# jiaozihao18/LC-Rec

Hardware: NVIDIA B200
Metric: items indexed/sec (4-level RQ + Sinkhorn collision resolution) (higher is better)
Workload: dtype f32

## Files before the change

include/lcrec_b200.h:

```cpp
#ifndef LCREC_B200_H
#define LCREC_B200_H

#include <stddef.h>
#include <stdint.h>

#ifdef __cplusplus
extern "C" {
#endif

#define LCREC_OK 0
#define LCREC_ERR_ARG 1
#define LCREC_ERR_CUDA 2
#define LCREC_ERR_UNSUPPORTED 3
#define LCREC_ERR_NOMEM 4
#define LCREC_ERR_NUMERIC 5

#define LCREC_MAX_LEVELS 8

int lcrec_version(void);
const char* lcrec_strerror(int code);
const char* lcrec_last_error(void);
int lcrec_device_check(void);

typedef struct lcrec_mlp lcrec_mlp_t;
// ... 135 lines not shown
                                        void* stream);
int lcrec_sort_codes(const int64_t* codes, int64_t n, int n_levels, const int32_t* n_codes,
                     uint64_t* keys_out, uint32_t* items_out, void* ws, int64_t ws_bytes, void* stream);

typedef struct lcrec_indexer lcrec_indexer_t;
int lcrec_indexer_create(lcrec_mlp_t* encoder, int e_dim, int n_levels, const float* const* codebooks,
                         const int32_t* n_codes, double last_epsilon, int sk_iters,
                         int64_t max_items, int64_t chunk_rows, lcrec_indexer_t** out);
int lcrec_indexer_destroy(lcrec_indexer_t* ix);
int lcrec_indexer_run_device(lcrec_indexer_t* ix, const float* x, int64_t n, int max_rounds,
                             int64_t* codes, int64_t* stats_host, void* stream);
int lcrec_indexer_run_host(lcrec_indexer_t* ix, const float* x_host, int64_t n, int max_rounds,
                           int64_t* codes_host, int64_t* stats_host, void* stream);
int lcrec_indexer_run_device_ex(lcrec_indexer_t* ix, const void* x, int dtype, int64_t n, int max_rounds,
                                int64_t* codes, int64_t* stats_host, void* stream);
int lcrec_indexer_run_host_ex(lcrec_indexer_t* ix, const void* x_host, int dtype, int64_t n, int max_rounds,
                              int64_t* codes_host, int64_t* stats_host, void* stream);
int lcrec_indexer_pass0(lcrec_indexer_t* ix, const float* x, int64_t n, int64_t row_offset, void* stream);
int lcrec_indexer_pass0_ex(lcrec_indexer_t* ix, const void* x, int dtype, int64_t n, int64_t row_offset, void* stream);
int lcrec_indexer_round(lcrec_indexer_t* ix, int64_t n, int64_t* counts_host, void* stream);
int lcrec_indexer_resolve(lcrec_indexer_t* ix, int64_t* codes, const float* resid, int64_t n, int max_rounds,
                          int64_t* stats_host, void* stream);
int lcrec_indexer_set_segments(int on);
int lcrec_indexer_set_speculative(int on);
int64_t* lcrec_indexer_codes(lcrec_indexer_t* ix);
float* lcrec_indexer_resid(lcrec_indexer_t* ix);
int64_t lcrec_kmeans_workspace_bytes(int64_t n, int e_dim, int n_codes);
int lcrec_kmeans_center(const float* x, int64_t n, int e_dim, float* xc, float* mean, double* mean_variance_host,
                        void* workspace, int64_t workspace_bytes, void* stream);
int lcrec_kmeans_lloyd(const float* xc, int64_t n, int e_dim, float* centers, int n_codes, int max_iter, double tol,
                       const float* add_mean, int64_t* labels_out, double* inertia_host, int* n_iter_host,
                       void* workspace, int64_t workspace_bytes, void* stream);
int64_t lcrec_kmeanspp_workspace_bytes(int64_t n, int n_trials);
int lcrec_kmeanspp_seed(const float* xc, int64_t n, int e_dim, int n_clusters, int64_t first_index, const double* draws,
                        int n_trials, int64_t* indices, float* centers, void* workspace, int64_t workspace_bytes,
                        void* stream);
int lcrec_ema_update(const float* latent, const int64_t* indices, int64_t n, int n_codes, int e_dim,
                     double ema_decay, double epsilon, float* cluster_size, float* ema_w, float* codebook,
                     void* stream);
int lcrec_codebook_usage(const float* cluster_size, int n_codes, double epsilon, double reset_threshold,
                         int64_t* used_codes, uint8_t* unused_mask, void* stream);
int64_t lcrec_masked_mean_pool_workspace_bytes(int64_t n_seq, int64_t seq_len, int hidden_dim);
int lcrec_masked_mean_pool(const void* hidden, int dtype, const int64_t* mask, int64_t n_seq, int64_t seq_len,
                           int hidden_dim, float* out, int64_t out_stride, int accumulate, double divide_by,
                           void* workspace, int64_t workspace_bytes, void* stream);
int64_t lcrec_index_json_workspace_bytes(int64_t n);
// ... 25 lines not shown
```

lcrec_b200/_lib.py:

```python
from __future__ import annotations

import ctypes as C
import os

_HERE = os.path.dirname(os.path.abspath(__file__))
LIB_PATH = os.path.join(_HERE, "liblcrec_b200.so")

i32, i64, f64 = C.c_int32, C.c_int64, C.c_double
vp = C.c_void_p
pp = C.POINTER(C.c_void_p)

SIGNATURES = {
    "lcrec_version": (C.c_int, []),
    "lcrec_strerror": (C.c_char_p, [C.c_int]),
    "lcrec_last_error": (C.c_char_p, []),
    "lcrec_device_check": (C.c_int, []),
    "lcrec_launch_count": (i64, []),
    "lcrec_mlp_create": (C.c_int, [C.c_int, C.POINTER(i32), pp, pp, C.c_int, vp, pp]),
    "lcrec_mlp_update": (C.c_int, [vp, pp, pp, vp]),
    "lcrec_mlp_destroy": (C.c_int, [vp]),
    "lcrec_mlp_workspace_bytes": (i64, [vp, i64]),
    "lcrec_mlp_forward": (C.c_int, [vp, vp, i64, vp, pp, vp, i64, vp]),
    "lcrec_mlp_forward_ex": (C.c_int, [vp, vp, C.c_int, i64, vp, pp, vp, i64, vp]),
    "lcrec_mlp_set_acc_chunk": (C.c_int, [vp, C.c_int]),
# ... 31 lines not shown
                                           C.c_int, C.c_int, C.c_int, vp, vp, i64, vp]),
    "lcrec_sinkhorn_set_mode": (C.c_int, [C.c_int]),
    "lcrec_collisions_workspace_bytes": (i64, [i64]),
    "lcrec_collisions": (C.c_int, [vp, i64, C.c_int, C.POINTER(i32), vp, vp, vp, vp, i64, vp]),
    "lcrec_sort_codes": (C.c_int, [vp, i64, C.c_int, C.POINTER(i32), vp, vp, vp, i64, vp]),
    "lcrec_prefix_segments": (C.c_int, [vp, i64, C.c_int, C.POINTER(i32), vp, vp, vp, vp, i64, vp]),
    "lcrec_segment_collisions_workspace_bytes": (i64, [i64]),
    "lcrec_collisions_in_segments": (C.c_int, [vp, i64, C.c_int, C.c_int, vp, vp, vp, i64, vp, vp, vp, vp, i64, vp]),
    "lcrec_collisions_in_segments_active": (C.c_int, [vp, i64, C.c_int, C.c_int, vp, vp, vp, i64, vp, vp, vp, vp, vp, vp, vp, vp,
                                                      i64, vp]),
    "lcrec_profile_enable": (C.c_int, [C.c_int]),
    "lcrec_profile_collect": (C.c_int, [C.POINTER(C.c_double), C.POINTER(i64)]),
    "lcrec_indexer_create": (C.c_int, [vp, C.c_int, C.c_int, pp, C.POINTER(i32), f64, C.c_int, i64, i64, pp]),
    "lcrec_indexer_destroy": (C.c_int, [vp]),
    "lcrec_indexer_run_device": (C.c_int, [vp, vp, i64, C.c_int, vp, C.POINTER(i64), vp]),
    "lcrec_indexer_run_host": (C.c_int, [vp, vp, i64, C.c_int, vp, C.POINTER(i64), vp]),
    "lcrec_indexer_pass0": (C.c_int, [vp, vp, i64, i64, vp]),
    "lcrec_indexer_run_device_ex": (C.c_int, [vp, vp, C.c_int, i64, C.c_int, vp, C.POINTER(i64), vp]),
    "lcrec_indexer_run_host_ex": (C.c_int, [vp, vp, C.c_int, i64, C.c_int, vp, C.POINTER(i64), vp]),
    "lcrec_indexer_pass0_ex": (C.c_int, [vp, vp, C.c_int, i64, i64, vp]),
    "lcrec_indexer_round": (C.c_int, [vp, i64, C.POINTER(i64), vp]),
    "lcrec_indexer_resolve": (C.c_int, [vp, vp, vp, i64, C.c_int, C.POINTER(i64), vp]),
    "lcrec_indexer_set_segments": (C.c_int, [C.c_int]),
    "lcrec_indexer_set_speculative": (C.c_int, [C.c_int]),
    "lcrec_ema_update": (C.c_int, [vp, vp, i64, C.c_int, C.c_int, f64, f64, vp, vp, vp, vp]),
    "lcrec_codebook_usage": (C.c_int, [vp, C.c_int, f64, f64, vp, vp, vp]),
    "lcrec_masked_mean_pool_workspace_bytes": (i64, [i64, i64, C.c_int]),
    "lcrec_masked_mean_pool": (C.c_int, [vp, C.c_int, vp, i64, i64, C.c_int, vp, i64, C.c_int, f64, vp, i64, vp]),
    "lcrec_kmeans_workspace_bytes": (i64, [i64, C.c_int, C.c_int]),
    "lcrec_kmeans_center": (C.c_int, [vp, i64, C.c_int, vp, vp, C.POINTER(f64), vp, i64, vp]),
    "lcrec_kmeans_lloyd": (C.c_int, [vp, i64, C.c_int, vp, C.c_int, C.c_int, f64, vp, vp, C.POINTER(f64), C.POINTER(C.c_int),
                                     vp, i64, vp]),
    "lcrec_rq_train_forward": (C.c_int, [vp, vp, i64, C.c_int, C.c_int, pp, vp, vp, vp, vp, vp]),
    "lcrec_rq_train_backward": (C.c_int, [vp, vp, i64, C.c_int, C.c_int, C.POINTER(i32), vp, vp, f64, vp, pp, vp]),
    "lcrec_adam_workspace_bytes": (i64, [C.c_int, C.POINTER(i64)]),
    "lcrec_adam_clip_step": (C.c_int, [C.c_int, pp, pp, pp, pp, C.POINTER(i64), f64, f64, f64, f64, f64, C.c_int, i64, f64,
                                       C.c_int, vp, vp, i64, vp]),
    "lcrec_adam_hyper": (C.c_int, [f64, f64, f64, f64, i64, C.POINTER(C.c_float)]),
    "lcrec_adam_clip_step_dev": (C.c_int, [C.c_int, pp, pp, pp, pp, C.POINTER(i64), vp, f64, f64, f64, f64, C.c_int, f64,
                                           C.c_int, vp, vp, i64, vp]),
    "lcrec_simple_opt_clip_step": (C.c_int, [C.c_int, C.c_int, pp, pp, pp, C.POINTER(i64), f64, f64, f64, f64, f64, C.c_int, vp, vp, i64, vp]),
    "lcrec_bn_sums_elems": (i64, [C.c_int]),
    "lcrec_bn_splits": (C.c_int, [i64, C.c_int]),
    "lcrec_bn_forward_reduce": (C.c_int, [vp, i64, C.c_int, vp, vp]),
    "lcrec_bn_forward_apply": (C.c_int, [vp, vp, C.c_int, i64, i64, C.c_int, vp, vp, f64, f64, C.c_int, vp, vp, vp, vp, vp, vp]),
    "lcrec_bn_backward_reduce": (C.c_int, [vp, vp, vp, C.c_int, vp, vp, i64, C.c_int, vp, vp]),
# ... 64 lines not shown
```

lcrec_b200/build.py:

```python
from __future__ import annotations

import os
import subprocess
import sys

HERE = os.path.dirname(os.path.abspath(__file__))
CSRC = os.path.join(HERE, "csrc")
LIB = os.path.join(HERE, "liblcrec_b200.so")
SOURCES = ["abi.cu", "linear_tf32x3.cu", "linear_pair.cu", "rq_fused.cu", "sinkhorn.cu", "collide.cu", "ema.cu", "pool.cu", "kmeans.cu", "rq_train.cu", "optim.cu", "kmeanspp.cu", "train_extra.cu", "json_emit.cu", "sinkhorn_cluster.cu", "exchange.cu"]
NVCC_FLAGS = ["-O3", "-std=c++17", "-gencode", "arch=compute_100a,code=sm_100a", "-lineinfo",
              "-Xcompiler", "-fPIC", "--expt-relaxed-constexpr"]


def _stale() -> bool:
    if not os.path.exists(LIB):
        return True
    t = os.path.getmtime(LIB)
    deps = [os.path.join(CSRC, f) for f in os.listdir(CSRC)] + [os.path.join(HERE, "..", "include", "lcrec_b200.h")]
    return any(os.path.getmtime(d) > t for d in deps)


def build(force: bool = False, verbose: bool = False) -> str:
    if not force and not _stale():
        return LIB
    nvcc = os.environ.get("NVCC", "/usr/local/cuda/bin/nvcc")
    objs = []
    procs = []
    for src in SOURCES:
        obj = os.path.join(CSRC, src.replace(".cu", ".o"))
        objs.append(obj)
        cmd = [nvcc, *NVCC_FLAGS, "-c", os.path.join(CSRC, src), "-o", obj]
        if verbose:
# ... 19 lines not shown
```

lcrec_b200/csrc/abi.cu:

```cuda
#include <stdarg.h>
#include <string.h>

#include <utility>
#include <vector>

#include <nvtx3/nvToolsExt.h>

#include "common.cuh"

namespace lcrec {

static const char* stage_name(int tag) {
  static const char* mlp[] = {"lcrec/mlp_layer1", "lcrec/mlp_layer2", "lcrec/mlp_layer3", "lcrec/mlp_layer4", "lcrec/mlp_layer5",
                              "lcrec/mlp_layer6", "lcrec/mlp_layer7", "lcrec/mlp_layer8+"};
  if (tag == 0) return "lcrec/input_operand_split";
  if (tag >= 1 && tag <= 16) return mlp[tag - 1 < 7 ? tag - 1 : 7];
  switch (tag) {
    case 17: return "lcrec/tail_operand_splits";
    case 20: return "lcrec/rq_quantize";
    case 21: return "lcrec/collision_check";
    case 22: return "lcrec/sinkhorn_groups_round1";
    case 23: return "lcrec/sinkhorn_groups_later_rounds";
    case 24: return "lcrec/sinkhorn_warp_classes";
    case 26: return "lcrec/sinkhorn_literal_rerun";
    default: return "lcrec/stage";
  }
}

static thread_local char g_err[512] = "";
std::atomic<int64_t> g_launches{0};

void set_error(const char* fmt, ...) {
  va_list ap;
  va_start(ap, fmt);
  vsnprintf(g_err, sizeof(g_err), fmt, ap);
  va_end(ap);
}

int num_sms() {
  static int sms = -1;
  if (sms < 0) {
// ... 91 lines not shown
  lcrec_mlp_t* enc = nullptr;
  int in_dim = 0, D = 0, L = 0;
  std::vector<const float*> cb;
  std::vector<int32_t> K;
  double eps = 0.003; int iters = 50;
  int64_t max_items = 0, chunk_rows = 0;
  int64_t* codes = nullptr; float* resid = nullptr; float* z = nullptr;
  void* mlp_ws = nullptr; int64_t mlp_ws_bytes = 0;
  int64_t* offsets = nullptr; int64_t* members = nullptr; int64_t* counts = nullptr; int32_t* flags = nullptr;
  void* col_ws = nullptr; int64_t col_ws_bytes = 0;
  void* sk_ws = nullptr; int64_t sk_ws_bytes = 0;
  int64_t* seg_offsets = nullptr; int64_t* seg_members = nullptr; int64_t* seg_counts = nullptr;
  void* seg_ws = nullptr; int64_t seg_ws_bytes = 0;
  int32_t* seg_active[2] = {nullptr, nullptr}; int32_t* seg_active_count = nullptr;
  float* stage[2] = {nullptr, nullptr};
  int64_t* counts_host = nullptr;
  cudaStream_t copy_stream = nullptr;
  cudaEvent_t ev_copied[2] = {nullptr, nullptr}, ev_consumed[2] = {nullptr, nullptr};
  cudaStream_t round_stream = nullptr; cudaEvent_t round_ev = nullptr;
  cudaGraphExec_t round_exec[2] = {nullptr, nullptr};
  int64_t round_launches[2] = {0, 0};
  const int64_t* rg_codes = nullptr; const float* rg_resid = nullptr; int64_t rg_n = -1; int rg_key = -1;
  bool rg_failed = false;
};

extern "C" int lcrec_mlp_in_dim(const lcrec_mlp_t* m);
extern "C" int lcrec_mlp_out_dim(const lcrec_mlp_t* m);

#define IX_ALLOC(ptr, bytes)                                                                     \
  do {                                                                                           \
    if (cudaMalloc((void**)&(ptr), (size_t)(bytes)) != cudaSuccess) {                            \
      set_error("indexer: cudaMalloc(%lld) failed: %s", (long long)(bytes), cudaGetErrorString(cudaGetLastError())); \
      lcrec_indexer_destroy(ix);                                                                 \
      return LCREC_ERR_NOMEM;                                                                    \
    }                                                                                            \
  } while (0)

extern "C" int lcrec_indexer_create(lcrec_mlp_t* encoder, int e_dim, int n_levels, const float* const* codebooks,
                                    const int32_t* n_codes, double last_epsilon, int sk_iters, int64_t max_items,
                                    int64_t chunk_rows, lcrec_indexer_t** out) {
  LC_ARG(encoder && e_dim > 0 && n_levels >= 1 && n_levels <= LCREC_MAX_LEVELS && codebooks && n_codes && out);
  LC_ARG(max_items > 0 && chunk_rows > 0 && last_epsilon > 0.0 && sk_iters >= 0);
  LC_ARG(lcrec_mlp_out_dim(encoder) == e_dim);
  LC_TRY(lcrec_device_check());
  lcrec_indexer* ix = new lcrec_indexer();
  ix->enc = encoder; ix->in_dim = lcrec_mlp_in_dim(encoder); ix->D = e_dim; ix->L = n_levels;
// ... 4 lines not shown
  IX_ALLOC(ix->resid, sizeof(float) * max_items * e_dim);
  IX_ALLOC(ix->z, sizeof(float) * max_items * e_dim);
  ix->mlp_ws_bytes = lcrec_mlp_workspace_bytes(encoder, ix->chunk_rows);
  IX_ALLOC(ix->mlp_ws, ix->mlp_ws_bytes);
  IX_ALLOC(ix->offsets, sizeof(int64_t) * (max_items + 1));
  IX_ALLOC(ix->members, sizeof(int64_t) * max_items);
  IX_ALLOC(ix->counts, sizeof(int64_t) * 8);
  ix->flags = reinterpret_cast<int32_t*>(ix->counts + 4);
  ix->col_ws_bytes = lcrec_collisions_workspace_bytes(max_items);
  IX_ALLOC(ix->col_ws, ix->col_ws_bytes);
  ix->sk_ws_bytes = lcrec_sinkhorn_groups_workspace_bytes(max_items, n_codes[n_levels - 1]);
  IX_ALLOC(ix->sk_ws, ix->sk_ws_bytes);
  IX_ALLOC(ix->seg_offsets, sizeof(int64_t) * (max_items + 1));
  IX_ALLOC(ix->seg_members, sizeof(int64_t) * max_items);
  IX_ALLOC(ix->seg_counts, sizeof(int64_t) * 8);
  ix->seg_ws_bytes = lcrec_segment_collisions_workspace_bytes(max_items / 2 + 1);
  IX_ALLOC(ix->seg_ws, ix->seg_ws_bytes);
  IX_ALLOC(ix->seg_active[0], sizeof(int32_t) * (max_items / 2 + 2));
  IX_ALLOC(ix->seg_active[1], sizeof(int32_t) * (max_items / 2 + 2));
  IX_ALLOC(ix->seg_active_count, sizeof(int32_t) * 2);
  if (cudaMallocHost((void**)&ix->counts_host, sizeof(int64_t) * 8) != cudaSuccess) {
    set_error("indexer: cudaMallocHost failed"); lcrec_indexer_destroy(ix); return LCREC_ERR_NOMEM;
  }
  *out = ix;
  return LCREC_OK;
}

extern "C" int lcrec_indexer_destroy(lcrec_indexer_t* ix) {
  if (!ix) return LCREC_OK;
  cudaFree(ix->codes); cudaFree(ix->resid); cudaFree(ix->z); cudaFree(ix->mlp_ws); cudaFree(ix->offsets);
  cudaFree(ix->members); cudaFree(ix->counts); cudaFree(ix->col_ws); cudaFree(ix->sk_ws);
  cudaFree(ix->seg_offsets); cudaFree(ix->seg_members); cudaFree(ix->seg_counts); cudaFree(ix->seg_ws);
  cudaFree(ix->seg_active[0]); cudaFree(ix->seg_active[1]); cudaFree(ix->seg_active_count);
  cudaFree(ix->stage[0]); cudaFree(ix->stage[1]);
  if (ix->counts_host) cudaFreeHost(ix->counts_host);
  for (int i = 0; i < 2; ++i) { if (ix->ev_copied[i]) cudaEventDestroy(ix->ev_copied[i]); if (ix->ev_consumed[i]) cudaEventDestroy(ix->ev_consumed[i]); }
  if (ix->copy_stream) cudaStreamDestroy(ix->copy_stream);
  for (int i = 0; i < 2; ++i) if (ix->round_exec[i]) cudaGraphExecDestroy(ix->round_exec[i]);
  if (ix->round_ev) cudaEventDestroy(ix->round_ev);
  if (ix->round_stream) cudaStreamDestroy(ix->round_stream);
  delete ix;
  return LCREC_OK;
}

extern "C" int64_t* lcrec_indexer_codes(lcrec_indexer_t* ix) { return ix ? ix->codes : nullptr; }
extern "C" float* lcrec_indexer_resid(lcrec_indexer_t* ix) { return ix ? ix->resid : nullptr; }

extern "C" int lcrec_indexer_pass0_ex(lcrec_indexer_t* ix, const void* x, int dtype, int64_t n, int64_t row_offset, void* stream) {
  LC_ARG(dtype_ok(dtype));
  LC_ARG(ix && n >= 0 && row_offset >= 0 && row_offset + n <= ix->max_items);
  if (n == 0) return LCREC_OK;
  LC_ARG(x != nullptr);
  const int64_t row_bytes = dtype_bytes(dtype) * ix->in_dim;
  for (int64_t s = 0; s < n; s += ix->chunk_rows) {
    const int64_t m = std::min(ix->chunk_rows, n - s);
    LC_TRY(lcrec_mlp_forward_ex(ix->enc, static_cast<const char*>(x) + s * row_bytes, dtype, m, ix->z + s * ix->D, nullptr,
                                ix->mlp_ws, ix->mlp_ws_bytes, stream));
  }
  {
    ProfScope prof(20, (cudaStream_t)stream);
    LC_TRY(lcrec_rq_quantize(ix->z, n, ix->D, ix->L, ix->cb.data(), ix->K.data(), ix->L, ix->L - 1,
                             ix->codes + row_offset * ix->L, nullptr, ix->resid + row_offset * ix->D,
                             nullptr, stream));
  }
  return LCREC_OK;
}

extern "C" int lcrec_indexer_pass0(lcrec_indexer_t* ix, const float* x, int64_t n, int64_t row_offset, void* stream) {
  return lcrec_indexer_pass0_ex(ix, x, kDtypeF32, n, row_offset, stream);
}

static int g_use_segments = 1;
extern "C" int lcrec_indexer_set_segments(int on) { g_use_segments = on ? 1 : 0; return LCREC_OK; }

static int collide_and_fetch(lcrec_indexer_t* ix, const int64_t* codes, int64_t n, int seg_round, cudaStream_t st) {
  {
    ProfScope prof(21, st);
    if (seg_round >= 0) {
      const int in = (seg_round + 1) & 1, out = seg_round & 1;
      LC_CUDA(cudaMemsetAsync(ix->seg_active_count + out, 0, sizeof(int32_t), st));
      LC_TRY(lcrec_collisions_in_segments_active(codes, n, ix->L, ix->L - 1, ix->seg_offsets, ix->seg_members, ix->seg_counts + 1,
                                                 n / 2 + 1, seg_round > 0 ? ix->seg_active[in] : nullptr,
// ... 254 lines not shown
```

lcrec_b200/csrc/common.cuh:

```cuda
#pragma once
#include <cuda_runtime.h>
#include <stdint.h>
#include <stdio.h>
#include <atomic>

#include "../../include/lcrec_b200.h"

namespace lcrec {

void set_error(const char* fmt, ...);
extern std::atomic<int64_t> g_launches;

inline void count_launch(int n = 1) { g_launches.fetch_add(n, std::memory_order_relaxed); }

#define LC_CUDA(expr)                                                                        \
  do {                                                                                       \
    cudaError_t _e = (expr);                                                                 \
    if (_e != cudaSuccess) {                                                                 \
      lcrec::set_error("%s failed: %s (%s:%d)", #expr, cudaGetErrorString(_e), __FILE__, __LINE__); \
      (void)cudaGetLastError();                                                              \
      return LCREC_ERR_CUDA;                                                                 \
    }                                                                                        \
  } while (0)

// ... 10 lines not shown
#define LC_ARG(cond)                                                                         \
  do {                                                                                       \
    if (!(cond)) {                                                                           \
      lcrec::set_error("bad argument: %s (%s:%d)", #cond, __FILE__, __LINE__);               \
      return LCREC_ERR_ARG;                                                                  \
    }                                                                                        \
  } while (0)

#define LC_TRY(expr)                                                                         \
  do {                                                                                       \
    int _r = (expr);                                                                         \
    if (_r != LCREC_OK) return _r;                                                           \
  } while (0)

constexpr int kDtypeF32 = 0, kDtypeF16 = 1, kDtypeBF16 = 2;
inline bool dtype_ok(int dtype) { return dtype == kDtypeF32 || dtype == kDtypeF16 || dtype == kDtypeBF16; }
inline int64_t dtype_bytes(int dtype) { return dtype == kDtypeF32 ? 4 : 2; }

inline int64_t round_up(int64_t x, int64_t m) { return (x + m - 1) / m * m; }
inline int64_t ceil_div(int64_t x, int64_t m) { return (x + m - 1) / m; }

int num_sms();

constexpr int kProfTags = 32;
void prof_begin(int tag, cudaStream_t st);
void prof_end(int tag, cudaStream_t st);
struct ProfScope {
  int tag; cudaStream_t st;
  ProfScope(int t, cudaStream_t s) : tag(t), st(s) { prof_begin(tag, st); }
  ~ProfScope() { prof_end(tag, st); }
};

struct Arena {
  char* base; int64_t size; int64_t off;
  Arena(void* p, int64_t n) : base((char*)p), size(n), off(0) {}
  template <typename T> T* take(int64_t count) {
    int64_t start = round_up(off, 256);
    int64_t end = start + (int64_t)sizeof(T) * count;
    if (end > size || base == nullptr) { off = size + 1; return nullptr; }
    off = end;
    return (T*)(base + start);
  }
  bool ok() const { return off <= size; }
};
inline int64_t arena_need(int64_t bytes) { return round_up(bytes, 256) + 256; }

// ... 2 lines not shown
```

lcrec_b200/csrc/linear_tf32x3.cu:

```cuda
#include <cuda.h>
#include <cuda_fp16.h>

#include <mutex>
#include <vector>

#include "common.cuh"
#include "linear.cuh"
#include "sm100_ptx.cuh"

namespace lcrec {

using namespace ptx;

struct LinearArgs {
  int64_t n_rows;
  int n_out;
  int num_kblocks;
  int chunk_kblocks;
  int relu;
  const float* bias;
  float* y;
  int64_t ldy;
  float* y_hi;
  float* y_lo;
// ... 529 lines not shown
                     arena_need(sizeof(float) * n_rows * ld4(hid)) + arena_need(sizeof(float) * n_rows) +
                     arena_need(sizeof(float) * n_rows * n_scale_groups(m->dims[0])) + 2 * arena_need(sizeof(float) * n_rows * n_scale_groups(hid));
  return std::max(tf, hf) + 1024;
}

static int mlp_forward_f16(lcrec_mlp_t* m, const void* x, int dtype, int64_t n_rows, float* y, float* const* acts, void* workspace,
                           int64_t workspace_bytes, cudaStream_t st) {
  Arena ar(workspace, workspace_bytes);
  const int64_t ld0 = ld8(m->dims[0]);
  const int64_t hid = std::max(m->max_hidden, 8);
  __half* in_hi = ar.take<__half>(n_rows * ld0);
  __half* in_lo = ar.take<__half>(n_rows * ld0);
  __half* set_hi[2]; __half* set_lo[2]; float* set_scale[2];
  for (int i = 0; i < 2; ++i) { set_hi[i] = ar.take<__half>(n_rows * ld8(hid)); set_lo[i] = ar.take<__half>(n_rows * ld8(hid)); }
  float* ybuf = ar.take<float>(n_rows * ld4(hid));
  float* rscale = ar.take<float>(n_rows);
  float* in_scale = ar.take<float>(n_rows * n_scale_groups(m->dims[0]));
  for (int i = 0; i < 2; ++i) set_scale[i] = ar.take<float>(n_rows * n_scale_groups(hid));
  if (!ar.ok()) { set_error("mlp_forward: workspace too small (%lld bytes given, %lld needed)", (long long)workspace_bytes, (long long)lcrec_mlp_workspace_bytes(m, n_rows)); return LCREC_ERR_NOMEM; }
  const bool allow_pair = !(m->variant & 16);
  auto pair_ok = [&](int l) { return allow_pair && l < m->n_layers && linear_pair_supported(m->dims[l], m->dims[l + 1], kPairGroup); };
  const void* cur = x; int cur_dtype = dtype; int64_t ldc = m->dims[0];
  SplitOperand grp{}; bool grouped = false; int next_set = 0;
  for (int l = 0; l < m->n_layers; ++l) {
    const bool last = (l == m->n_layers - 1);
    const int k = m->dims[l], n_out = m->dims[l + 1];
    float* act_out = (acts && acts[l]) ? acts[l] : nullptr;
    if (pair_ok(l)) {
      if (!grouped) {
        ProfScope prof(l == 0 ? 0 : 17, st);
        __half* hi = l == 0 ? in_hi : set_hi[next_set];
        __half* lo = l == 0 ? in_lo : set_lo[next_set];
        float* sc = l == 0 ? in_scale : set_scale[next_set];
        if (l != 0) next_set ^= 1;
        LC_TRY(launch_split_groups(cur, cur_dtype, n_rows, k, ldc, hi, lo, ld8(k), sc, n_rows, st));
        grp.hi = hi; grp.lo = lo; grp.ld = ld8(k); grp.inv_scale = sc; grp.ld_scale = n_rows; grp.group = kPairGroup;
        grouped = true;
      }
      PairProblem p{};
      p.a = grp; p.n_rows = n_rows; p.k = k;
      p.w_hi = m->h_hi[l]; p.w_lo = m->h_lo[l]; p.ldw = m->ldh[l]; p.w_inv_scale = m->h_scale[l];
      p.n_out = n_out; p.bias = m->bias[l]; p.relu = last ? m->relu_last : 1;
      p.debug = ((m->variant >> 2) & 3) | ((m->variant & 32) ? 4 : 0) | ((m->variant & 64) ? 8 : 0);
      if (l == 0) p.trace = m->trace;
      const bool next_pair = !last && pair_ok(l + 1);
      if (next_pair) {
        p.o_hi = set_hi[next_set]; p.o_lo = set_lo[next_set]; p.ldo = ld8(n_out);
        p.o_inv_scale = set_scale[next_set]; p.ld_oscale = n_rows;
      }
      if (last) { p.y = y; p.ldy = n_out; }
      else if (act_out) { p.y = act_out; p.ldy = n_out; }
      else if (!next_pair) { p.y = ybuf; p.ldy = ld4(n_out); }
      { ProfScope prof(1 + std::min(l, 15), st); LC_TRY(launch_linear_pair(p, st)); }
      if (next_pair) {
        grp.hi = p.o_hi; grp.lo = p.o_lo; grp.ld = p.ldo; grp.inv_scale = p.o_inv_scale; grp.ld_scale = n_rows; grp.group = kPairGroup;
        next_set ^= 1;
      } else {
        grouped = false; cur = p.y; cur_dtype = kDtypeF32; ldc = p.ldy;
      }
      continue;
    }
    {
      ProfScope prof(l == 0 ? 0 : 17, st);
      LC_TRY(launch_split_f16_ex(cur, cur_dtype, n_rows, k, ldc, l == 0 ? in_hi : set_hi[0], l == 0 ? in_lo : set_lo[0], ld8(k), rscale, st));
    }
    LinearProblem p{};
    p.f16 = true; p.row_scale = rscale; p.col_scale = m->h_scale[l];
    p.a_hi = l == 0 ? in_hi : set_hi[0]; p.a_lo = l == 0 ? in_lo : set_lo[0]; p.n_rows = n_rows; p.k = k; p.lda = ld8(k);
    p.w_hi = m->h_hi[l]; p.w_lo = m->h_lo[l]; p.n_out = n_out; p.ldw = m->ldh[l];
    p.bias = m->bias[l]; p.relu = last ? m->relu_last : 1;
    p.acc_chunk = m->acc_chunk; p.variant = m->variant & 15;
    float* out = last ? y : (act_out ? act_out : ybuf);
    const int64_t ldo = last ? n_out : (act_out ? n_out : ld4(n_out));
    p.y = out; p.ldy = ldo;
    if ((p.ldy & 3) || (reinterpret_cast<uintptr_t>(p.y) & 15)) {
      set_error("mlp_forward: output width %lld must be a multiple of 4 floats and 16-byte aligned", (long long)p.ldy);
      return LCREC_ERR_UNSUPPORTED;
    }
    { ProfScope prof(1 + std::min(l, 15), st); LC_TRY(launch_linear(p, st)); }
    cur = out; cur_dtype = kDtypeF32; ldc = ldo;
  }
  if (acts && acts[m->n_layers - 1] && acts[m->n_layers - 1] != y)
    LC_CUDA(cudaMemcpyAsync(acts[m->n_layers - 1], y, sizeof(float) * n_rows * m->dims[m->n_layers], cudaMemcpyDeviceToDevice, st));
  return LCREC_OK;
}

extern "C" int lcrec_mlp_forward(lcrec_mlp_t* m, const float* x, int64_t n_rows, float* y, float* const* acts,
                                 void* workspace, int64_t workspace_bytes, void* stream) {
  return lcrec_mlp_forward_ex(m, x, kDtypeF32, n_rows, y, acts, workspace, workspace_bytes, stream);
}

// ... 265 lines not shown
```

lcrec_b200/csrc/rq_fused.cu:

```cuda
#include <cuda_fp16.h>

#include "common.cuh"
#include "linear.cuh"

namespace lcrec {

constexpr int kRqThreads = 256;

struct RqArgs {
  const float* z; int64_t n; int n_levels; int n_levels_run; int resid_level;
  const float* cb[LCREC_MAX_LEVELS]; int k[LCREC_MAX_LEVELS];
  int64_t* codes; float* xq; float* resid_last; double* sq_err;
};

__device__ __forceinline__ double block_sum_double(double v, double* scratch) {
  for (int o = 16; o > 0; o >>= 1) v += __shfl_xor_sync(0xffffffffu, v, o);
  const int warp = threadIdx.x >> 5, lane = threadIdx.x & 31;
  if (lane == 0) scratch[warp] = v;
  __syncthreads();
  double t = 0.0;
  if (warp == 0) {
    t = lane < (blockDim.x >> 5) ? scratch[lane] : 0.0;
    for (int o = 16; o > 0; o >>= 1) t += __shfl_xor_sync(0xffffffffu, t, o);
  }
// ... 452 lines not shown
static int launch_rq_smem(const RqArgs& a, size_t smem, cudaStream_t st) {
  if (a.xq != nullptr || a.sq_err != nullptr) return launch_rq_smem_impl<D, 1, true, 256>(a, smem, st);
  if constexpr (D <= 32) {
    if (a.n >= 4096) {
      if (g_rq_ipt == 4 && a.n >= 65536) return launch_rq_smem_impl<D, 4, false, 256>(a, smem, st);
      return launch_rq_smem_impl<D, 2, false, 512>(a, smem, st);
    }
  }
  return launch_rq_smem_impl<D, 1, false, 256>(a, smem, st);
}

}

using namespace lcrec;

static int g_rq_tc_mode = 1;
extern "C" int lcrec_rq_set_tc_mode(int mode) {
  if (mode == 12 || mode == 14) { g_rq_ipt = mode - 10; return LCREC_OK; }
  LC_ARG(mode >= 0 && mode <= 2);
  g_rq_tc_mode = mode;
  return LCREC_OK;
}

extern "C" int lcrec_rq_quantize(const float* z, int64_t n, int e_dim, int n_levels, const float* const* codebooks,
                                 const int32_t* n_codes, int n_levels_run, int resid_level, int64_t* codes,
                                 float* xq, float* resid_last, double* sq_err, void* stream) {
  LC_ARG(n >= 0 && e_dim > 0 && n_levels >= 1 && n_levels <= LCREC_MAX_LEVELS && codebooks && n_codes);
  LC_ARG(n_levels_run >= 0 && n_levels_run <= n_levels);
  LC_TRY(lcrec_device_check());
  if (n == 0) return LCREC_OK;
  LC_ARG(z != nullptr);
  cudaStream_t st = (cudaStream_t)stream;
  RqArgs a{};
  a.z = z; a.n = n; a.n_levels = n_levels; a.n_levels_run = n_levels_run; a.resid_level = resid_level;
  a.codes = codes; a.xq = xq; a.resid_last = resid_last; a.sq_err = sq_err;
  size_t smem = 0; int64_t total_codes = 0;
  for (int l = 0; l < n_levels; ++l) {
    LC_ARG(codebooks[l] != nullptr && n_codes[l] > 0);
    a.cb[l] = codebooks[l]; a.k[l] = n_codes[l];
    if (l < n_levels_run) { smem += sizeof(float) * ((size_t)n_codes[l] * e_dim + ((n_codes[l] + 3) & ~3)); total_codes += n_codes[l]; }
  }
  const bool aligned = (reinterpret_cast<uintptr_t>(z) & 15) == 0 && (!xq || (reinterpret_cast<uintptr_t>(xq) & 15) == 0) &&
                       (!resid_last || (reinterpret_cast<uintptr_t>(resid_last) & 15) == 0);
  bool cb_aligned = true;
  for (int l = 0; l < n_levels_run; ++l) cb_aligned = cb_aligned && (reinterpret_cast<uintptr_t>(codebooks[l]) & 15) == 0;
  bool tc_ok = codes != nullptr && n_levels_run > 0 && g_rq_tc_mode != 0 && n >= 1024, tc_big = false;
// ... 37 lines not shown
```

lcrec_b200/ops.py:

```python
from __future__ import annotations

import ctypes as C
from typing import List, Optional, Sequence, Tuple

import torch

from . import _lib


def _stream(t: torch.Tensor) -> C.c_void_p:
    return C.c_void_p(torch.cuda.current_stream(t.device).cuda_stream)


def _need_cuda(*ts: torch.Tensor) -> None:
    for t in ts:
        if t is not None and not t.is_cuda:
            raise RuntimeError("lcrec_b200 operators run on a CUDA (sm_100a) device only; there is no CPU "
                               f"fallback (got a tensor on {t.device})")


def _f32c(t: torch.Tensor) -> torch.Tensor:
    return t.detach().to(torch.float32).contiguous()


# ... 606 lines not shown
    c = codes.detach().to(torch.int64).contiguous()
    n, L = c.shape
    dev = c.device
    level = L - 1 if level is None else level
    offsets = torch.empty((n + 1,), dtype=torch.int64, device=dev)
    members = torch.empty((max(n, 1),), dtype=torch.int64, device=dev)
    counts = torch.zeros((8,), dtype=torch.int64, device=dev)
    max_segs = segs["n_segments"]
    ws = _ws(lib.lcrec_segment_collisions_workspace_bytes(max_segs), dev)
    with torch.cuda.device(dev):
        _lib.check(lib.lcrec_collisions_in_segments(_p(c), n, L, int(level), _p(segs["offsets"]), _p(segs["members"]),
                                                    _p(segs["counts_dev"][1:2]), max_segs, _p(offsets), _p(members),
                                                    _p(counts), _p(ws), ws.numel(), _stream(c)))
    vals = [int(v) for v in counts.tolist()]
    n_unique, n_groups, n_rows, max_mult = vals[:4]
    return {"offsets": offsets[: n_groups + 1], "members": members[:n_rows], "n_unique": n_unique, "n_groups": n_groups,
            "n_rows": n_rows, "max_multiplicity": max_mult, "counts_dev": counts, "fallback": bool(vals[5])}


def indexer_set_segments(on: bool) -> None:
    _lib.check(_lib.load().lcrec_indexer_set_segments(int(bool(on))))


def indexer_set_speculative(mode) -> None:
    _lib.check(_lib.load().lcrec_indexer_set_speculative(2 if mode is True else int(mode)))


def sort_codes(codes: torch.Tensor, n_codes: Sequence[int]):
    _need_cuda(codes)
    lib = _lib.load()
    c = codes.detach().to(torch.int64).contiguous()
    n, L = c.shape
    keys = torch.empty((n,), dtype=torch.int64, device=c.device)
    items = torch.empty((n,), dtype=torch.int32, device=c.device)
    ws = _ws(lib.lcrec_collisions_workspace_bytes(n), c.device)
    with torch.cuda.device(c.device):
        _lib.check(lib.lcrec_sort_codes(_p(c), n, L, _lib.i32_array(n_codes), _p(keys), _p(items), _p(ws), ws.numel(),
                                        _stream(c)))
    return keys, items


def sinkhorn_groups(resid: torch.Tensor, codebook: torch.Tensor, offsets: torch.Tensor, members: torch.Tensor,
                    n_groups_dev: torch.Tensor, max_groups: int, max_rows: int, epsilon: float, iters: int,
                    codes: torch.Tensor, level: int, part_mod: int = 1, part_rem: int = 0, want_risky: bool = False):
    _need_cuda(resid, codebook, offsets, members, codes)
    lib = _lib.load()
# ... 149 lines not shown
```

Baseline: 13.92 million.

## Fuse all RQ levels into one 2-SM tcgen05 kernel with split-f16 codebooks

Adds a persistent 2-CTA cluster kernel that runs all residual-quantization levels in one launch. Distances come from split hi/lo f16 UMMA into tensor memory, and residuals stay in registers between levels. Codebooks are pre-split and their norms precomputed once at indexer creation. The MLP tail also hands its split f16 rows straight to the last layer, so a separate split pass is skipped. The trade is added complexity and a three-term f16 split approximation of fp32 distances, which could flip argmin ties compared with the old path.

```diff
diff --git a/include/lcrec_b200.h b/include/lcrec_b200.h
--- a/include/lcrec_b200.h
+++ b/include/lcrec_b200.h
@@ -181,6 +181,7 @@
 int lcrec_indexer_resolve(lcrec_indexer_t* ix, int64_t* codes, const float* resid, int64_t n, int max_rounds,
                           int64_t* stats_host, void* stream);
 int lcrec_indexer_set_segments(int on);
+int lcrec_indexer_set_rq_fused(int on);
 int lcrec_indexer_set_speculative(int on);
 int64_t* lcrec_indexer_codes(lcrec_indexer_t* ix);
 float* lcrec_indexer_resid(lcrec_indexer_t* ix);
diff --git a/lcrec_b200/_lib.py b/lcrec_b200/_lib.py
--- a/lcrec_b200/_lib.py
+++ b/lcrec_b200/_lib.py
@@ -77,6 +77,7 @@
     "lcrec_indexer_round": (C.c_int, [vp, i64, C.POINTER(i64), vp]),
     "lcrec_indexer_resolve": (C.c_int, [vp, vp, vp, i64, C.c_int, C.POINTER(i64), vp]),
     "lcrec_indexer_set_segments": (C.c_int, [C.c_int]),
+    "lcrec_indexer_set_rq_fused": (C.c_int, [C.c_int]),
     "lcrec_indexer_set_speculative": (C.c_int, [C.c_int]),
     "lcrec_ema_update": (C.c_int, [vp, vp, i64, C.c_int, C.c_int, f64, f64, vp, vp, vp, vp]),
     "lcrec_codebook_usage": (C.c_int, [vp, C.c_int, f64, f64, vp, vp, vp]),
diff --git a/lcrec_b200/build.py b/lcrec_b200/build.py
--- a/lcrec_b200/build.py
+++ b/lcrec_b200/build.py
@@ -7,7 +7,7 @@
 HERE = os.path.dirname(os.path.abspath(__file__))
 CSRC = os.path.join(HERE, "csrc")
 LIB = os.path.join(HERE, "liblcrec_b200.so")
-SOURCES = ["abi.cu", "linear_tf32x3.cu", "linear_pair.cu", "rq_fused.cu", "sinkhorn.cu", "collide.cu", "ema.cu", "pool.cu", "kmeans.cu", "rq_train.cu", "optim.cu", "kmeanspp.cu", "train_extra.cu", "json_emit.cu", "sinkhorn_cluster.cu", "exchange.cu"]
+SOURCES = ["abi.cu", "linear_tf32x3.cu", "linear_pair.cu", "rq_fused.cu", "rq_pair.cu", "sinkhorn.cu", "collide.cu", "ema.cu", "pool.cu", "kmeans.cu", "rq_train.cu", "optim.cu", "kmeanspp.cu", "train_extra.cu", "json_emit.cu", "sinkhorn_cluster.cu", "exchange.cu"]
 NVCC_FLAGS = ["-O3", "-std=c++17", "-gencode", "arch=compute_100a,code=sm_100a", "-lineinfo",
               "-Xcompiler", "-fPIC", "--expt-relaxed-constexpr"]
 
diff --git a/lcrec_b200/csrc/abi.cu b/lcrec_b200/csrc/abi.cu
--- a/lcrec_b200/csrc/abi.cu
+++ b/lcrec_b200/csrc/abi.cu
@@ -17,6 +17,7 @@
   if (tag >= 1 && tag <= 16) return mlp[tag - 1 < 7 ? tag - 1 : 7];
   switch (tag) {
     case 17: return "lcrec/tail_operand_splits";
+    case 18: return "lcrec/rq_levels_fused";
     case 20: return "lcrec/rq_quantize";
     case 21: return "lcrec/collision_check";
     case 22: return "lcrec/sinkhorn_groups_round1";
@@ -154,6 +155,7 @@
   int64_t round_launches[2] = {0, 0};
   const int64_t* rg_codes = nullptr; const float* rg_resid = nullptr; int64_t rg_n = -1; int rg_key = -1;
   bool rg_failed = false;
+  void* rq_books = nullptr;
 };
 
 extern "C" int lcrec_mlp_in_dim(const lcrec_mlp_t* m);
@@ -204,6 +206,18 @@
   if (cudaMallocHost((void**)&ix->counts_host, sizeof(int64_t) * 8) != cudaSuccess) {
     set_error("indexer: cudaMallocHost failed"); lcrec_indexer_destroy(ix); return LCREC_ERR_NOMEM;
   }
+  bool cb_aligned = true;
+  for (int l = 0; l < n_levels; ++l) cb_aligned = cb_aligned && (reinterpret_cast<uintptr_t>(codebooks[l]) & 15) == 0;
+  if (cb_aligned && rq_levels_pair_supported(e_dim, n_levels, n_codes)) {
+    IX_ALLOC(ix->rq_books, rq_levels_pair_books_bytes(n_levels));
+    int rc = cudaDeviceSynchronize() == cudaSuccess ? rq_levels_pair_prepare(codebooks, n_levels, ix->rq_books, 0) : LCREC_ERR_CUDA;
+    if (rc == LCREC_OK && cudaDeviceSynchronize() != cudaSuccess) rc = LCREC_ERR_CUDA;
+    if (rc != LCREC_OK) {
+      if (rc == LCREC_ERR_CUDA) set_error("indexer: codebook preparation failed: %s", cudaGetErrorString(cudaGetLastError()));
+      lcrec_indexer_destroy(ix);
+      return rc;
+    }
+  }
   *out = ix;
   return LCREC_OK;
 }
@@ -214,7 +228,7 @@
   cudaFree(ix->members); cudaFree(ix->counts); cudaFree(ix->col_ws); cudaFree(ix->sk_ws);
   cudaFree(ix->seg_offsets); cudaFree(ix->seg_members); cudaFree(ix->seg_counts); cudaFree(ix->seg_ws);
   cudaFree(ix->seg_active[0]); cudaFree(ix->seg_active[1]); cudaFree(ix->seg_active_count);
-  cudaFree(ix->stage[0]); cudaFree(ix->stage[1]);
+  cudaFree(ix->stage[0]); cudaFree(ix->stage[1]); cudaFree(ix->rq_books);
   if (ix->counts_host) cudaFreeHost(ix->counts_host);
   for (int i = 0; i < 2; ++i) { if (ix->ev_copied[i]) cudaEventDestroy(ix->ev_copied[i]); if (ix->ev_consumed[i]) cudaEventDestroy(ix->ev_consumed[i]); }
   if (ix->copy_stream) cudaStreamDestroy(ix->copy_stream);
@@ -227,6 +241,9 @@
 
 extern "C" int64_t* lcrec_indexer_codes(lcrec_indexer_t* ix) { return ix ? ix->codes : nullptr; }
 extern "C" float* lcrec_indexer_resid(lcrec_indexer_t* ix) { return ix ? ix->resid : nullptr; }
+
+static int g_rq_levels_fused = 1;
+extern "C" int lcrec_indexer_set_rq_fused(int on) { g_rq_levels_fused = on ? 1 : 0; return LCREC_OK; }
 
 extern "C" int lcrec_indexer_pass0_ex(lcrec_indexer_t* ix, const void* x, int dtype, int64_t n, int64_t row_offset, void* stream) {
   LC_ARG(dtype_ok(dtype));
@@ -239,7 +256,11 @@
     LC_TRY(lcrec_mlp_forward_ex(ix->enc, static_cast<const char*>(x) + s * row_bytes, dtype, m, ix->z + s * ix->D, nullptr,
                                 ix->mlp_ws, ix->mlp_ws_bytes, stream));
   }
-  {
+  if (ix->rq_books && g_rq_levels_fused && n >= rq_tc_min_rows()) {
+    ProfScope prof(18, (cudaStream_t)stream);
+    LC_TRY(launch_rq_levels_pair(ix->z, n, ix->L, ix->rq_books, ix->codes + row_offset * ix->L,
+                                 ix->resid + row_offset * ix->D, ix->L - 1, (cudaStream_t)stream));
+  } else {
     ProfScope prof(20, (cudaStream_t)stream);
     LC_TRY(lcrec_rq_quantize(ix->z, n, ix->D, ix->L, ix->cb.data(), ix->K.data(), ix->L, ix->L - 1,
                              ix->codes + row_offset * ix->L, nullptr, ix->resid + row_offset * ix->D,
diff --git a/lcrec_b200/csrc/common.cuh b/lcrec_b200/csrc/common.cuh
--- a/lcrec_b200/csrc/common.cuh
+++ b/lcrec_b200/csrc/common.cuh
@@ -56,6 +56,13 @@
 
 int num_sms();
 
+bool rq_levels_pair_supported(int e_dim, int n_levels, const int32_t* n_codes);
+int64_t rq_levels_pair_books_bytes(int n_levels);
+int rq_levels_pair_prepare(const float* const* codebooks, int n_levels, void* books, cudaStream_t st);
+int launch_rq_levels_pair(const float* z, int64_t n, int n_levels, const void* books,
+                          int64_t* codes, float* resid, int resid_level, cudaStream_t st);
+int64_t rq_tc_min_rows();
+
 constexpr int kProfTags = 32;
 void prof_begin(int tag, cudaStream_t st);
 void prof_end(int tag, cudaStream_t st);
diff --git a/lcrec_b200/csrc/linear_tf32x3.cu b/lcrec_b200/csrc/linear_tf32x3.cu
--- a/lcrec_b200/csrc/linear_tf32x3.cu
+++ b/lcrec_b200/csrc/linear_tf32x3.cu
@@ -575,6 +575,7 @@
   auto pair_ok = [&](int l) { return allow_pair && l < m->n_layers && linear_pair_supported(m->dims[l], m->dims[l + 1], kPairGroup); };
   const void* cur = x; int cur_dtype = dtype; int64_t ldc = m->dims[0];
   SplitOperand grp{}; bool grouped = false; int next_set = 0;
+  const __half *row_hi = nullptr, *row_lo = nullptr;
   for (int l = 0; l < m->n_layers; ++l) {
     const bool last = (l == m->n_layers - 1);
     const int k = m->dims[l], n_out = m->dims[l + 1];
@@ -597,29 +598,33 @@
       p.debug = ((m->variant >> 2) & 3) | ((m->variant & 32) ? 4 : 0) | ((m->variant & 64) ? 8 : 0);
       if (l == 0) p.trace = m->trace;
       const bool next_pair = !last && pair_ok(l + 1);
-      if (next_pair) {
+      const bool hand_rows = !last && !next_pair && n_out <= kPairGroup;
+      if (next_pair || hand_rows) {
         p.o_hi = set_hi[next_set]; p.o_lo = set_lo[next_set]; p.ldo = ld8(n_out);
-        p.o_inv_scale = set_scale[next_set]; p.ld_oscale = n_rows;
+        p.o_inv_scale = next_pair ? set_scale[next_set] : rscale; p.ld_oscale = n_rows;
       }
       if (last) { p.y = y; p.ldy = n_out; }
       else if (act_out) { p.y = act_out; p.ldy = n_out; }
-      else if (!next_pair) { p.y = ybuf; p.ldy = ld4(n_out); }
+      else if (!next_pair && !hand_rows) { p.y = ybuf; p.ldy = ld4(n_out); }
       { ProfScope prof(1 + std::min(l, 15), st); LC_TRY(launch_linear_pair(p, st)); }
       if (next_pair) {
         grp.hi = p.o_hi; grp.lo = p.o_lo; grp.ld = p.ldo; grp.inv_scale = p.o_inv_scale; grp.ld_scale = n_rows; grp.group = kPairGroup;
         next_set ^= 1;
       } else {
         grouped = false; cur = p.y; cur_dtype = kDtypeF32; ldc = p.ldy;
+        if (hand_rows) { row_hi = p.o_hi; row_lo = p.o_lo; }
       }
       continue;
     }
-    {
+    if (row_hi == nullptr) {
       ProfScope prof(l == 0 ? 0 : 17, st);
       LC_TRY(launch_split_f16_ex(cur, cur_dtype, n_rows, k, ldc, l == 0 ? in_hi : set_hi[0], l == 0 ? in_lo : set_lo[0], ld8(k), rscale, st));
+      row_hi = l == 0 ? in_hi : set_hi[0]; row_lo = l == 0 ? in_lo : set_lo[0];
     }
     LinearProblem p{};
     p.f16 = true; p.row_scale = rscale; p.col_scale = m->h_scale[l];
-    p.a_hi = l == 0 ? in_hi : set_hi[0]; p.a_lo = l == 0 ? in_lo : set_lo[0]; p.n_rows = n_rows; p.k = k; p.lda = ld8(k);
+    p.a_hi = row_hi; p.a_lo = row_lo; p.n_rows = n_rows; p.k = k; p.lda = ld8(k);
+    row_hi = row_lo = nullptr;
     p.w_hi = m->h_hi[l]; p.w_lo = m->h_lo[l]; p.n_out = n_out; p.ldw = m->ldh[l];
     p.bias = m->bias[l]; p.relu = last ? m->relu_last : 1;
     p.acc_chunk = m->acc_chunk; p.variant = m->variant & 15;
diff --git a/lcrec_b200/csrc/rq_fused.cu b/lcrec_b200/csrc/rq_fused.cu
--- a/lcrec_b200/csrc/rq_fused.cu
+++ b/lcrec_b200/csrc/rq_fused.cu
@@ -498,6 +498,8 @@
   return LCREC_OK;
 }
 
+int64_t lcrec::rq_tc_min_rows() { return g_rq_tc_mode == 0 ? INT64_MAX : (g_rq_tc_mode == 2 ? 1024 : 4096); }
+
 extern "C" int lcrec_rq_quantize(const float* z, int64_t n, int e_dim, int n_levels, const float* const* codebooks,
                                  const int32_t* n_codes, int n_levels_run, int resid_level, int64_t* codes,
                                  float* xq, float* resid_last, double* sq_err, void* stream) {
diff --git a/lcrec_b200/csrc/rq_pair.cu b/lcrec_b200/csrc/rq_pair.cu
--- /dev/null
+++ b/lcrec_b200/csrc/rq_pair.cu
@@ -0,0 +1,293 @@
+#include <cuda.h>
+#include <cuda_fp16.h>
+
+#include <algorithm>
+
+#include "linear.cuh"
+#include "sm100_ptx.cuh"
+
+namespace lcrec {
+
+using namespace ptx;
+
+namespace {
+
+constexpr int kD = 32;
+constexpr int kCodes = 256;
+constexpr int kRows = 128;
+constexpr int kThreads = 512;
+constexpr int kRowBytes = kD * 2;
+constexpr int kSlab = kRows * kRowBytes;
+constexpr uint32_t kSbo = 8 * kRowBytes;
+constexpr uint32_t kLayout = 4;
+constexpr int kMaxLevels = 4;
+
+constexpr int kOffA = kMaxLevels * 2 * kSlab;
+constexpr int kOffF = kOffA + 2 * kSlab;
+constexpr int kFloats = kMaxLevels * 2 * kCodes + 2 * kRows + 8 * kRows;
+constexpr int kOffBar = kOffF + kFloats * 4;
+constexpr int kSmemBytes = kOffBar + 64 + 1024;
+static_assert(kSmemBytes <= 232448, "shared memory");
+
+struct RqPairArgs {
+  const float* z; int64_t n; int levels; int resid_level;
+  const float* cb;
+  const __half* w_hi; const __half* w_lo;
+  const float* w_sc; const float* cc;
+  int64_t* codes; float* resid;
+};
+
+__device__ __forceinline__ uint32_t sw64(int r, int c) { return (uint32_t)(r * kRowBytes + ((c ^ ((r >> 1) & 3)) << 4)); }
+
+__global__ void __cluster_dims__(2, 1, 1) __launch_bounds__(kThreads, 1) rq_levels_pair_kernel(const RqPairArgs a) {
+  extern __shared__ uint8_t smem_raw[];
+  const uint32_t raw = smem_u32(smem_raw);
+  const uint32_t base = (raw + 1023u) & ~1023u;
+  uint8_t* smem = smem_raw + (base - raw);
+  float* fs = reinterpret_cast<float*>(smem + kOffF);
+  float* s_cs = fs;
+  float* s_cn = fs + kMaxLevels * kCodes;
+  float* s_xx = fs + 2 * kMaxLevels * kCodes;
+  float* s_sc = s_xx + kRows;
+  float* s_best = s_sc + kRows;
+  int* s_idx = reinterpret_cast<int*>(s_best + 4 * kRows);
+  const uint32_t a_full = base + kOffBar;
+  const uint32_t t_full = base + kOffBar + 8;
+  const uint32_t tmem_slot = base + kOffBar + 16;
+  volatile uint32_t* tmem_slot_ptr = reinterpret_cast<volatile uint32_t*>(smem + kOffBar + 16);
+
+  const int warp = threadIdx.x >> 5, lane = threadIdx.x & 31;
+  const uint32_t rank = cluster_ctarank();
+  const int64_t cluster_id = blockIdx.x >> 1, n_clusters = gridDim.x >> 1;
+  const int64_t n_units = (a.n + 2 * kRows - 1) / (2 * kRows);
+  const int L = a.levels;
+
+  if (threadIdx.x == 0) {
+    mbar_init(a_full, 8);
+    mbar_init(t_full, 1);
+    fence_barrier_init();
+  }
+  if (warp == 0) tmem_alloc_2sm(tmem_slot, 256);
+  for (int i = threadIdx.x; i < L * 2 * kRows * 4; i += kThreads) {
+    const int c = i & 3, r = (i >> 2) % kRows, hl = (i / (4 * kRows)) & 1, l = i / (8 * kRows);
+    const __half* src = (hl ? a.w_lo : a.w_hi) + ((size_t)l * kCodes + rank * kRows + r) * kD + c * 8;
+    *reinterpret_cast<uint4*>(smem + (l * 2 + hl) * kSlab + sw64(r, c)) = __ldg(reinterpret_cast<const uint4*>(src));
+  }
+  for (int i = threadIdx.x; i < L * kCodes; i += kThreads) {
+    s_cs[i] = __ldg(a.w_sc + i);
+    s_cn[i] = __ldg(a.cc + i);
+  }
+  fence_proxy_async();
+  tc_fence_before();
+  cluster_sync_all();
+  tc_fence_after();
+  const uint32_t tmem_base = *tmem_slot_ptr;
+
+  {
+    const int q = warp & 3, cq = warp >> 2;
+    const int rr = q * 32 + lane;
+    const bool owner = cq == 0;
+    const uint32_t t_addr = tmem_base + ((uint32_t)(q * 32) << 16) + (uint32_t)(cq * 64);
+    const uint32_t a_full_leader = a_full & kPeerBitMask;
+    constexpr uint32_t idesc = umma_idesc(256, kCodes, 0);
+    const uint64_t d_ahi = umma_smem_desc(base + kOffA, kSbo, kLayout);
+    const uint64_t d_alo = umma_smem_desc(base + kOffA + kSlab, kSbo, kLayout);
+    float v[kD];
+    uint32_t it = 0;
+    for (int64_t unit = cluster_id; unit < n_units; unit += n_clusters) {
+      const int64_t row = unit * (2 * kRows) + rank * kRows + rr;
+      const bool row_ok = row < a.n;
+      if (owner) {
+        const float4* zp = reinterpret_cast<const float4*>(a.z + (row_ok ? row : 0) * kD);
+#pragma unroll
+        for (int d = 0; d < kD / 4; ++d) {
+          const float4 t = row_ok ? __ldcs(zp + d) : make_float4(0.f, 0.f, 0.f, 0.f);
+          v[4 * d] = t.x; v[4 * d + 1] = t.y; v[4 * d + 2] = t.z; v[4 * d + 3] = t.w;
+        }
+      }
+      for (int l = 0; l < L; ++l, ++it) {
+        if (owner) {
+          if (l == a.resid_level && row_ok) {
+            float4* rp = reinterpret_cast<float4*>(a.resid + row * kD);
+#pragma unroll
+            for (int d = 0; d < kD / 4; ++d) rp[d] = make_float4(v[4 * d], v[4 * d + 1], v[4 * d + 2], v[4 * d + 3]);
+          }
+          float xx = 0.f, m = 0.f;
+#pragma unroll
+          for (int d = 0; d < kD; ++d) { xx = fmaf(v[d], v[d], xx); m = fmaxf(m, fabsf(v[d])); }
+          float s = 1.f, is = 1.f;
+          if (m > 0.f && m < INFINITY) {
+            int e;
+            frexpf(m, &e);
+            const int sh = min(max(15 - e, -100), 100);
+            s = ldexpf(1.f, sh); is = ldexpf(1.f, -sh);
+          }
+          s_xx[rr] = xx; s_sc[rr] = is;
+#pragma unroll
+          for (int c = 0; c < 4; ++c) {
+            uint32_t wh[4], wl[4];
+#pragma unroll
+            for (int i = 0; i < 4; ++i) {
+              uint32_t hh[2], ll[2];
+#pragma unroll
+              for (int j = 0; j < 2; ++j) {
+                const float xs = v[8 * c + 2 * i + j] * s;
+                const __half h = __float2half_rn(xs);
+                hh[j] = __half_as_ushort(h);
+                ll[j] = __half_as_ushort(__float2half_rn(xs - __half2float(h)));
+              }
+              wh[i] = hh[0] | (hh[1] << 16); wl[i] = ll[0] | (ll[1] << 16);
+            }
+            *reinterpret_cast<uint4*>(smem + kOffA + sw64(rr, c)) = make_uint4(wh[0], wh[1], wh[2], wh[3]);
+            *reinterpret_cast<uint4*>(smem + kOffA + kSlab + sw64(rr, c)) = make_uint4(wl[0], wl[1], wl[2], wl[3]);
+          }
+          fence_proxy_async();
+        }
+        asm volatile("bar.sync 1, 512;" ::: "memory");
+        if (owner) {
+          __syncwarp();
+          if (lane == 0) mbar_arrive_cluster(a_full_leader);
+        }
+        if (rank == 0 && warp == 0 && lane == 0) {
+          mbar_wait(a_full, it & 1u);
+          tc_fence_after();
+          const uint64_t d_bhi = umma_smem_desc(base + (l * 2) * kSlab, kSbo, kLayout);
+          const uint64_t d_blo = umma_smem_desc(base + (l * 2 + 1) * kSlab, kSbo, kLayout);
+#pragma unroll
+          for (int k = 0; k < kD / 16; ++k) {
+            const uint64_t adv = (uint64_t)(k * 32 >> 4);
+            umma_f16_2sm(tmem_base, d_alo + adv, d_bhi + adv, idesc, k == 0 ? 0u : 1u);
+            umma_f16_2sm(tmem_base, d_ahi + adv, d_blo + adv, idesc, 1u);
+            umma_f16_2sm(tmem_base, d_ahi + adv, d_bhi + adv, idesc, 1u);
+          }
+          umma_commit_2sm(t_full, 3);
+        }
+        __syncwarp();
+        mbar_wait(t_full, it & 1u);
+        tc_fence_after();
+        const float sc = s_sc[rr], xr = s_xx[rr];
+        const float* cs_l = s_cs + l * kCodes + cq * 64;
+        const float* cn_l = s_cn + l * kCodes + cq * 64;
+        float best = INFINITY; int best_i = 0;
+        auto scan32 = [&](const uint32_t (&t)[32], int j0) {
+#pragma unroll
+          for (int j = 0; j < 32; j += 4) {
+            const float4 cs = *reinterpret_cast<const float4*>(cs_l + j0 + j);
+            const float4 cn = *reinterpret_cast<const float4*>(cn_l + j0 + j);
+            const float a0 = fmaf(__uint_as_float(t[j]), sc, 0.f), a1 = fmaf(__uint_as_float(t[j + 1]), sc, 0.f);
+            const float a2 = fmaf(__uint_as_float(t[j + 2]), sc, 0.f), a3 = fmaf(__uint_as_float(t[j + 3]), sc, 0.f);
+            const float d0 = (xr + cn.x) - 2.f * (a0 * cs.x), d1 = (xr + cn.y) - 2.f * (a1 * cs.y);
+            const float d2 = (xr + cn.z) - 2.f * (a2 * cs.z), d3 = (xr + cn.w) - 2.f * (a3 * cs.w);
+            const int col = cq * 64 + j0 + j;
+            if (d0 < best) { best = d0; best_i = col; }
+            if (d1 < best) { best = d1; best_i = col + 1; }
+            if (d2 < best) { best = d2; best_i = col + 2; }
+            if (d3 < best) { best = d3; best_i = col + 3; }
+          }
+        };
+#pragma unroll
+        for (int j0 = 0; j0 < 64; j0 += 32) {
+          uint32_t t[32];
+          tmem_ld32(t_addr + j0, t);
+          tmem_wait_ld();
+          scan32(t, j0);
+        }
+        tc_fence_before();
+        if (!owner) { s_best[cq * kRows + rr] = best; s_idx[cq * kRows + rr] = best_i; }
+        asm volatile("bar.sync 1, 512;" ::: "memory");
+        if (owner) {
+#pragma unroll
+          for (int o = 1; o < 4; ++o) {
+            const float ob = s_best[o * kRows + rr];
+            const int oi = s_idx[o * kRows + rr];
+            if (ob < best || (ob == best && oi < best_i)) { best = ob; best_i = oi; }
+          }
+          if (row_ok) a.codes[row * L + l] = (int64_t)best_i;
+          if (l + 1 < L) {
+            const float4* qp = reinterpret_cast<const float4*>(a.cb + ((size_t)l * kCodes + best_i) * kD);
+#pragma unroll
+            for (int d = 0; d < kD / 4; ++d) {
+              const float4 t4 = __ldg(qp + d);
+              const float qq[4] = {t4.x, t4.y, t4.z, t4.w};
+#pragma unroll
+              for (int e = 0; e < 4; ++e) {
+                const float t = qq[e] - v[4 * d + e];
+                const float xres = v[4 * d + e] + t;
+                v[4 * d + e] = v[4 * d + e] - xres;
+              }
+            }
+          }
+        }
+      }
+    }
+  }
+  tc_fence_before();
+  cluster_sync_all();
+  if (warp == 0) {
+    tc_fence_after();
+    tmem_dealloc_2sm(tmem_base, 256);
+  }
+}
+
+}
+
+bool rq_levels_pair_supported(int e_dim, int n_levels, const int32_t* n_codes) {
+  if (e_dim != kD || n_levels < 1 || n_levels > kMaxLevels) return false;
+  for (int l = 0; l < n_levels; ++l) if (n_codes[l] != kCodes) return false;
+  return true;
+}
+
+int64_t rq_levels_pair_books_bytes(int n_levels) {
+  return (int64_t)n_levels * kCodes * (kD * (int64_t)sizeof(float) + 2 * kD * (int64_t)sizeof(__half) + 2 * (int64_t)sizeof(float));
+}
+
+int launch_split_f16(const float* x, int64_t rows, int k, int64_t ldx, __half* hi, __half* lo, int64_t ld_out,
+                     float* inv_scale, cudaStream_t st);
+__global__ void code_norms_kernel(const float* __restrict__ cb, int k, int D, float* __restrict__ out);
+
+int rq_levels_pair_prepare(const float* const* codebooks, int n_levels, void* books, cudaStream_t st) {
+  float* cb = static_cast<float*>(books);
+  __half* hi = reinterpret_cast<__half*>(cb + (size_t)n_levels * kCodes * kD);
+  __half* lo = hi + (size_t)n_levels * kCodes * kD;
+  float* sc = reinterpret_cast<float*>(lo + (size_t)n_levels * kCodes * kD);
+  float* cc = sc + (size_t)n_levels * kCodes;
+  for (int l = 0; l < n_levels; ++l) {
+    LC_CUDA(cudaMemcpyAsync(cb + (size_t)l * kCodes * kD, codebooks[l], sizeof(float) * kCodes * kD, cudaMemcpyDeviceToDevice, st));
+    LC_TRY(launch_split_f16(codebooks[l], kCodes, kD, kD, hi + (size_t)l * kCodes * kD, lo + (size_t)l * kCodes * kD, kD,
+                            sc + l * kCodes, st));
+    code_norms_kernel<<<1, kCodes, 0, st>>>(codebooks[l], kCodes, kD, cc + l * kCodes);
+    LC_LAUNCH_CHECK("code_norms_kernel");
+  }
+  return LCREC_OK;
+}
+
+int launch_rq_levels_pair(const float* z, int64_t n, int n_levels, const void* books,
+                          int64_t* codes, float* resid, int resid_level, cudaStream_t st) {
+  if (n == 0) return LCREC_OK;
+  static int max_clusters = 0;
+  if (max_clusters == 0) {
+    LC_CUDA(cudaFuncSetAttribute(rq_levels_pair_kernel, cudaFuncAttributeMaxDynamicSharedMemorySize, kSmemBytes));
+    cudaLaunchConfig_t cfg{};
+    cfg.gridDim = dim3(2 * (unsigned)num_sms()); cfg.blockDim = dim3(kThreads); cfg.dynamicSmemBytes = kSmemBytes;
+    cudaLaunchAttribute at{};
+    at.id = cudaLaunchAttributeClusterDimension; at.val.clusterDim.x = 2; at.val.clusterDim.y = 1; at.val.clusterDim.z = 1;
+    cfg.attrs = &at; cfg.numAttrs = 1;
+    int c = 0;
+    if (cudaOccupancyMaxActiveClusters(&c, rq_levels_pair_kernel, &cfg) != cudaSuccess || c < 1) { (void)cudaGetLastError(); c = num_sms() / 2; }
+    max_clusters = c;
+  }
+  RqPairArgs a{};
+  a.z = z; a.n = n; a.levels = n_levels; a.resid_level = resid_level;
+  a.cb = static_cast<const float*>(books);
+  a.w_hi = reinterpret_cast<const __half*>(a.cb + (size_t)n_levels * kCodes * kD);
+  a.w_lo = a.w_hi + (size_t)n_levels * kCodes * kD;
+  a.w_sc = reinterpret_cast<const float*>(a.w_lo + (size_t)n_levels * kCodes * kD);
+  a.cc = a.w_sc + (size_t)n_levels * kCodes;
+  a.codes = codes; a.resid = resid;
+  const int64_t clusters = std::min<int64_t>(ceil_div(n, 2 * kRows), max_clusters);
+  rq_levels_pair_kernel<<<(unsigned)(2 * clusters), kThreads, kSmemBytes, st>>>(a);
+  LC_LAUNCH_CHECK("rq_levels_pair_kernel");
+  return LCREC_OK;
+}
+
+}
diff --git a/lcrec_b200/ops.py b/lcrec_b200/ops.py
--- a/lcrec_b200/ops.py
+++ b/lcrec_b200/ops.py
@@ -652,6 +652,10 @@
     _lib.check(_lib.load().lcrec_indexer_set_segments(int(bool(on))))
 
 
+def indexer_set_rq_fused(on: bool) -> None:
+    _lib.check(_lib.load().lcrec_indexer_set_rq_fused(int(bool(on))))
+
+
 def indexer_set_speculative(mode) -> None:
     _lib.check(_lib.load().lcrec_indexer_set_speculative(2 if mode is True else int(mode)))
 
```

New measurement: 13.95 million, median of 6. No clear change (+0.2%).
